# vnminin/phylomap

Hardware: AMD Instinct MI355X
Metric: stochastic-map realisations/sec (branches x sites sampled/s) (higher is better)
Workload: dtype f64; 1 GPU; C3: sumstatMCMC_bigtree sweep, 4-state Q, 10000-tip synthetic tree, Omega*mean(t_b)=4; n_states=4, n_tips=10000, branches=19998, replicas_total=16384, max_iters_provisioned=63, parallelism=replica-sharded x1 (weak), one RCCL all-reduce of the statistics

## Files before the change

### phylomap_amd/csrc/phm_device.h

```cpp
#pragma once

#include <hip/hip_runtime.h>
#include <stdint.h>

#define PHM_LOGTAB_QUAL __device__
#include "phm_logtab.h"

namespace phm {

constexpr uint32_t DERR_ZERO_PROB = 1u;
constexpr uint32_t DERR_CAPACITY  = 2u;
constexpr uint32_t DERR_UNIF_CAP  = 4u;
constexpr uint32_t DERR_SAMPLEONCE = 8u;

constexpr uint32_t ENT_NODE   = 0u;
constexpr uint32_t ENT_BSTATE = 1u << 30;
constexpr uint32_t ENT_BEXP   = 2u << 30;
constexpr uint32_t ENT_BUNIF  = 3u << 30;

#ifndef PHM_EXPERIMENT_PHILOX_ROUNDS
#define PHM_EXPERIMENT_PHILOX_ROUNDS 7
#endif
constexpr int PHILOX_ROUNDS = PHM_EXPERIMENT_PHILOX_ROUNDS;
__device__ __forceinline__ void philox4x32(uint32_t c0, uint32_t c1, uint32_t c2, uint32_t c3,
// ... 150 lines not shown
  for (int j = 1; j < NS - 1; ++j) { cum += p[j]; idx += (thr <= cum) ? 0 : 1; }
  return idx;
}

template <int NS>
__device__ __forceinline__ void matvec_u(const double* __restrict__ M, double (&v)[NS]) {
  double y[NS];
#pragma unroll
  for (int i = 0; i < NS; ++i) {
    double acc = M[i * NS] * v[0];
#pragma unroll
    for (int j = 1; j < NS; ++j) acc += M[i * NS + j] * v[j];
    y[i] = acc;
  }
#pragma unroll
  for (int i = 0; i < NS; ++i) v[i] = y[i];
}

template <int CTRL, int ROW_MASK>
__device__ __forceinline__ int dpp_max_step(int v) {
  const int o = __builtin_amdgcn_update_dpp(0, v, CTRL, ROW_MASK, 0xf, false);
  return o > v ? o : v;
}
__device__ __forceinline__ int wave_max_count(int v) {
  v = dpp_max_step<0x111, 0xf>(v);
  v = dpp_max_step<0x112, 0xf>(v);
  v = dpp_max_step<0x114, 0xf>(v);
  v = dpp_max_step<0x118, 0xf>(v);
  v = dpp_max_step<0x142, 0xa>(v);
  v = dpp_max_step<0x143, 0xc>(v);
  return __builtin_amdgcn_readlane(v, 63);
}

}
```

### phylomap_amd/csrc/phm_engine.cpp

```cpp
#include "phm_internal.h"

namespace {

int tree_levels(const phm::Schedule& s) {
  std::vector<int32_t> depth(s.n_node, 0);
  int levels = 1;
  for (const phm::DownStep& d : s.down)
    if (d.child >= 0) { depth[d.child] = depth[d.parent] + 1; levels = std::max(levels, depth[d.child] + 1); }
  return levels;
}
bool deep_tree(const phm::Schedule& s) {
  int lg2 = 0;
  while ((1 << lg2) < s.n_node + 1) ++lg2;
  return tree_levels(s) > 4 * lg2 + 32;
}

inline int narrow_auto_max_replicas(const phm::Schedule& s) {
  const int levels = tree_levels(s);
  const double E = (double)s.n_edge;
  const double cap = (0.0048 * levels + 6e-6 * E - 0.01) / (6.5e-7 * E);
  return (int)std::max(8.0, std::min(4096.0, cap));
}
constexpr int TILES_AUTO_MAX_REPLICAS = 262144;
inline int wbranch_auto_max_replicas(const phm::Schedule& s) {
// ... 514 lines not shown
    p.cnt = e->d_wb_cnt.as<double>(); p.rowbuf = e->d_nw_rowbuf.as<double>();
    p.dmap = e->d_nw_dmap.as<uint8_t>();
  }
  return PHM_OK;
}

inline int tiles_cnt_copies(int tiles) {
  int c = 1;
  while (c < 64 && c * tiles < 512) c *= 2;
  return c;
}

int32_t tiles_branch_group(int tiles, int n_edge) { return (int32_t)std::max<int64_t>(1, std::min<int64_t>(16, (int64_t)tiles * n_edge / 65536)); }

template <int NS>
void fill_tile_params(phm_engine* e, phm::TileParams<NS>& p, const phm_options& o) {
  fill_common(e, o, p);
  p.klong = e->nw_klong;
  p.tile0 = 0; p.tiles_part = e->tiles;
  p.group = tiles_branch_group(e->tiles, p.n_edge);
  p.n_groups = (p.n_edge + p.group - 1) / p.group;
  p.n_chunks = (p.n_groups + phm::TILES_CHUNK - 1) / phm::TILES_CHUNK;
  p.rows = e->nw_total_cap;
  p.up = e->d_up.as<phm::UpStep>();
  p.up_order = e->d_nw_up_order.as<int32_t>(); p.node_order = e->d_nw_node_order.as<int32_t>();
  p.branch_order = e->d_nw_border.as<int32_t>(); p.slot = e->d_tl_slot.as<int32_t>();
  p.cl_nodes = e->d_nw_cl_nodes.as<phm::ClusterNode>();
  p.cl_lvl_ptr = e->d_nw_cl_lvl_ptr.as<int32_t>(); p.cl_lvl_off = e->d_nw_cl_lvl_off.as<int32_t>();
  p.colL = e->d_nw_colL.as<double>(); p.rowL = e->d_nw_rowL.as<double>(); p.maskL = e->d_nw_maskL.as<double>();
  p.tips = e->d_tips.as<uint8_t>(); p.mcount = e->d_mcount.as<uint16_t>();
  p.dw[0] = e->d_dw0.as<double>(); p.dw[1] = e->d_dw1.as<double>();
  p.estate = e->d_tl_estate.as<uint8_t>(); p.PL = e->d_PL.as<double>(); p.nstate = e->d_nstate.as<uint8_t>();
  p.mstate = e->d_wt_mstate.p ? e->d_wt_mstate.as<uint8_t>() : nullptr;
  p.pdw = e->d_tl_pdw.as<double>(); p.pchunk = e->d_tl_pchunk.as<double>(); p.cnt = e->d_tl_cnt.as<uint32_t>();
  p.cnt_copies = tiles_cnt_copies(e->tiles);
  p.pseg = e->d_tl_pseg.as<uint32_t>(); p.segprev = e->d_tl_segprev.as<uint32_t>(); p.gseg = e->d_tl_gseg.p ? e->d_tl_gseg.as<uint32_t>() : nullptr;
}

int32_t tile_slots(phm_engine* e, const SlotPlan& sp) {
  const int E = e->sched.n_edge;
  e->tl_slot.assign(E + 1, 0);
  for (int b = 0; b < E; ++b) {
    if (sp.cap[b] >= (1 << 23)) return fail(PHM_ERR_UNSUPPORTED, "branch too long: a slot of the (tile, branch) mapping exceeds 4 GB");
    if (sp.off[b + 1] > 0x7fffff00ll / 64) return fail(PHM_ERR_UNSUPPORTED, "tree too large: dwell rows per replica tile exceed 32-bit indexing");
    e->tl_slot[b + 1] = (int32_t)sp.off[b + 1];
  }
  return PHM_OK;
}

int32_t tiles_setup(phm_engine* e, const phm_tree* x, const phm_model* model, const phm_options& o, int32_t max_iters) {
  const phm::Schedule& s = e->sched;
  const int E = s.n_edge, Nn = s.n_node, n = e->n, tiles = e->tiles;
  const SlotPlan sp = plan_slots(e, x, model->Omega, o, max_iters);
  if (int32_t st = tile_slots(e, sp)) return st;
  const int64_t rows = e->rows;
  single_tree_tips(e, x);

  const int n_chunks = (E + phm::TILES_CHUNK - 1) / phm::TILES_CHUNK;
  const size_t dw_bytes = sizeof(double) * (size_t)tiles * rows * 64;
  const size_t tab = (size_t)e->nw_klong * n * n;
  const size_t pdw_bytes = sizeof(double) * (size_t)tiles * E * n * 64;
  const size_t pl_bytes = sizeof(double) * (size_t)tiles * Nn * n * 64;
#ifndef PHM_TILES_LONG_SEGMENTS
#define PHM_TILES_LONG_SEGMENTS 48.0
#endif
  const bool long_paths = sp.max_seg > PHM_TILES_LONG_SEGMENTS;
  const size_t ms_bytes = long_paths ? (size_t)tiles * rows * 64 : 0;
  size_t free_b = 0, total_b = 0;
  HIPCHK(hipMemGetInfo(&free_b, &total_b));
  const int group = tiles_branch_group(tiles, E);
  const size_t gseg_bytes = group > 1 ? sizeof(uint32_t) * (size_t)tiles * ((E + group - 1) / group) * 64 : 0;
  const size_t need = 2 * dw_bytes + ms_bytes + pdw_bytes + gseg_bytes + pl_bytes + stats_bytes(e) + sizeof(double) * 3 * tab + (size_t)tiles * (4 * (size_t)E + Nn) * 64;
  if (int32_t st = check_hbm(need, free_b)) return st;
  HIPCHK(upload(e->d_up, s.up)); HIPCHK(upload(e->d_down, s.down));
  if (int32_t st = build_level_orders(e)) return st;
  HIPCHK(upload(e->d_nw_border, sp.order)); HIPCHK(upload(e->d_tl_slot, e->tl_slot));
  HIPCHK(e->d_nw_colL.alloc(sizeof(double) * tab)); HIPCHK(e->d_nw_rowL.alloc(sizeof(double) * tab));
  HIPCHK(e->d_nw_maskL.alloc(sizeof(double) * (size_t)e->nw_klong * 2 * n));
  HIPCHK(upload(e->d_tips, e->tips_host));
  HIPCHK(e->d_mcount.alloc(sizeof(uint16_t) * (size_t)tiles * E * 64));
  HIPCHK(e->d_dw0.alloc(dw_bytes)); HIPCHK(e->d_dw1.alloc(dw_bytes));
  if (long_paths) HIPCHK(e->d_wt_mstate.alloc(ms_bytes));
  HIPCHK(e->d_tl_estate.alloc((size_t)tiles * E * 64));
  HIPCHK(e->d_PL.alloc(pl_bytes));
  HIPCHK(e->d_nstate.alloc((size_t)tiles * Nn * 64));
  HIPCHK(e->d_tl_pdw.alloc(pdw_bytes));
  if (gseg_bytes) HIPCHK(e->d_tl_gseg.alloc(gseg_bytes));
  HIPCHK(e->d_tl_pchunk.alloc(sizeof(double) * (size_t)tiles * n_chunks * n * 64));
  HIPCHK(e->d_tl_cnt.alloc(sizeof(uint32_t) * (size_t)tiles * tiles_cnt_copies(tiles) * n * n * 64));
  HIPCHK(e->d_tl_pseg.alloc(sizeof(uint32_t) * (size_t)tiles * n_chunks * 64)); HIPCHK(e->d_tl_segprev.alloc(sizeof(uint32_t) * tiles));
  if (int32_t st = alloc_stats(e)) return st;
  e->bytes = (int64_t)(2 * dw_bytes + ms_bytes + pdw_bytes + gseg_bytes + pl_bytes + e->d_stats.bytes + e->d_red.bytes + e->d_mcount.bytes + e->d_tl_pchunk.bytes +
                       sizeof(double) * 3 * tab);
  HIPCHK(hipMemset(e->d_nstate.p, 0, e->d_nstate.bytes));
  HIPCHK(hipMemset(e->d_tl_cnt.p, 0, e->d_tl_cnt.bytes));
  if (int32_t st = init_tile_paths(e, x)) return st;
  {
    std::vector<uint32_t> segprev(tiles);
    for (int t = 0; t < tiles; ++t) segprev[t] = (uint32_t)((int64_t)x->map_off[E] * std::min(64, e->S - t * 64));
    HIPCHK(hipMemcpy(e->d_tl_segprev.p, segprev.data(), e->d_tl_segprev.bytes, hipMemcpyHostToDevice));
  }
  e->nw_tier_off.clear();
  const bool deep = deep_tree(s);
  if (e->dbg.level_groups >= 2 || (e->dbg.level_groups == 0 && (deep || (int64_t)tiles * Nn <= phm::TILES_CL_MAX_WORK))) {
    phm::ClusterPlan plan;
    if (e->dbg.level_groups == 3 || (e->dbg.level_groups == 0 && deep)) phm::build_cluster_plan(s, phm::TILES_CL_NODES, plan);
    else phm::build_band_plan(s, TILES_CL_BAND, plan);
    if (int32_t st = upload_cluster_plan(e, plan, false)) return st;
  }
  small_n(e, [&](auto& p) { fill_tile_params(e, p.tl, o); });
  return PHM_OK;
}

int32_t wtiles_setup(phm_engine* e, const phm_tree* x, const phm_model* model, const phm_options& o, int32_t max_iters) {
  const phm::Schedule& s = e->sched;
// ... 731 lines not shown
extern "C" {

int32_t phm_engine_dump(phm_engine* e, int32_t replica, int32_t* seg_count, double* seg_dwell, int32_t seg_cap,
                        int32_t* node_states, double* PL) {
  e = live(e);
  if (!e) return fail(PHM_ERR_STATE, "engine is NULL");
  if (e->dead) return dead_engine();
  if (replica < 0 || replica >= e->S) return fail(PHM_ERR_BAD_INPUT, "replica out of range");
  HIPCHK(hipSetDevice(e->device));
  HIPCHK(hipStreamSynchronize(e->last_stream));
  const bool branches = e->mapping == PHM_MAP_BRANCHES;
  const int padded = branches ? replica : e->pad_index(replica), L = branches ? 1 : 64, blk = padded / L, lane = padded % L;
  const phm::Schedule& s = e->scheds[e->n_trees > 1 ? blk / e->tpt : 0];
  const int E = s.n_edge, T = s.n_tips, n = e->n;
  if (branches) {
    std::vector<int32_t> mc(E);
    HIPCHK(hipMemcpy(mc.data(), e->d_nw_mcount.as<int32_t>() + (size_t)replica * E, sizeof(int32_t) * E, hipMemcpyDeviceToHost));
    if (seg_count) for (int b = 0; b < E; ++b) seg_count[b] = mc[b];
    if (seg_dwell) {
      std::vector<double> dw((size_t)e->nw_total_cap);
      const double* src = ((e->iters_done & 1) ? e->d_nw_dwB.as<double>() : e->d_nw_dwA.as<double>()) + (size_t)replica * e->nw_total_cap;
      HIPCHK(hipMemcpy(dw.data(), src, sizeof(double) * dw.size(), hipMemcpyDeviceToHost));
      for (int b = 0; b < E; ++b)
        for (int i = 0; i < std::min<int>(mc[b], seg_cap); ++i) seg_dwell[(size_t)b * seg_cap + i] = dw[(size_t)e->nw_off[b] + i];
    }
  } else {
    std::vector<uint16_t> mc((size_t)E * 64);
    HIPCHK(hipMemcpy(mc.data(), e->d_mcount.as<uint16_t>() + (size_t)blk * E * 64, sizeof(uint16_t) * mc.size(), hipMemcpyDeviceToHost));
    if (seg_count) for (int b = 0; b < E; ++b) seg_count[b] = mc[(size_t)b * 64 + lane];
    if (seg_dwell && e->mapping == PHM_MAP_TILES) {
      std::vector<double> dw((size_t)e->rows * 64);
      const double* src = ((e->iters_done & 1) ? e->d_dw1.as<double>() : e->d_dw0.as<double>()) + (size_t)blk * e->rows * 64;
      HIPCHK(hipMemcpy(dw.data(), src, sizeof(double) * dw.size(), hipMemcpyDeviceToHost));
      for (int b = 0; b < E; ++b)
        for (int i = 0; i < std::min<int>(mc[(size_t)b * 64 + lane], seg_cap); ++i)
          seg_dwell[(size_t)b * seg_cap + i] = dw[((size_t)e->tl_slot[b] + i) * 64 + lane];
    } else if (seg_dwell) {
      std::vector<double> dw((size_t)e->rows * 64);
      int32_t cur[2];
      HIPCHK(hipMemcpy(cur, e->d_cursor.as<int32_t>() + 2 * blk, sizeof cur, hipMemcpyDeviceToHost));
      const double* src = ((!e->ring && cur[0]) ? e->d_dw1.as<double>() : e->d_dw0.as<double>()) + (size_t)blk * e->rows * 64;
      HIPCHK(hipMemcpy(dw.data(), src, sizeof(double) * dw.size(), hipMemcpyDeviceToHost));
      size_t row = e->ring ? (size_t)cur[0] : 0;
      for (int k = 0; k < E; ++k) {
        const phm::DownStep& d = s.down[k];
        int m = std::min<int>(mc[(size_t)d.edge * 64 + lane], seg_cap);
        for (int i = 0; i < m; ++i) seg_dwell[(size_t)d.edge * seg_cap + i] = dw[((row + i) % (size_t)e->rows) * 64 + lane];
        int mx = 0;
        for (int l = 0; l < 64; ++l) mx = std::max<int>(mx, mc[(size_t)d.edge * 64 + l]);
        row += mx;
      }
    }
  }
  auto tip_state = [&](int t) -> int { return e->tips_per_replica ? e->tips_host[((size_t)blk * T + t) * L + lane] : e->tips_host[t]; };
  if (node_states) {
    std::vector<uint8_t> ns((size_t)s.n_node * L);
    HIPCHK(hipMemcpy(ns.data(), e->d_nstate.as<uint8_t>() + (size_t)blk * s.n_node * L, ns.size(), hipMemcpyDeviceToHost));
    for (int t = 0; t < T; ++t) node_states[t] = tip_state(t) + 1;
    for (int v = 0; v < s.n_node; ++v) node_states[T + v] = ns[(size_t)v * L + lane] + 1;
  }
  if (PL) {
    std::vector<double> pl((size_t)s.n_node * n * L);
    HIPCHK(hipMemcpy(pl.data(), e->d_PL.as<double>() + (size_t)blk * s.n_node * n * L, sizeof(double) * pl.size(), hipMemcpyDeviceToHost));
    for (int t = 0; t < T; ++t)
      for (int c = 0; c < n; ++c) PL[(size_t)t * n + c] = (c == tip_state(t)) ? 1.0 : 0.0;
    for (int v = 0; v < s.n_node; ++v)
      for (int c = 0; c < n; ++c)
        PL[(size_t)(T + v) * n + c] = (e->wide() && e->mapping == PHM_MAP_REPLICAS) ? pl[((size_t)v * L + lane) * n + c] : pl[((size_t)v * n + c) * L + lane];
  }
// ... 92 lines not shown
```

### phylomap_amd/csrc/phm_internal.h

```cpp
#pragma once

#include "../../include/phylomap_hip.h"

#include <hip/hip_runtime.h>

#include <algorithm>
#include <cmath>
#include <cstdio>
#include <chrono>
#include <cstdlib>
#include <cstring>
#include <memory>
#include <string>
#include <thread>
#include <vector>

#include "phm_exp.h"
#include "phm_mcmc.h"
#include "phm_mcmc_maps.h"
#include "phm_narrow.h"
#include "phm_qupdate.h"
#include "phm_sched.h"
#include "phm_tiles.h"
#include "phm_wbranch.h"
// ... 260 lines not shown
  bool recover = true;
  int recoveries = 0;
  bool dead = false;
  int n = 0, cols = 0, dcols = 0, variant = 0;
  std::vector<double> qparams;
  std::vector<std::vector<double>> qhist;
  double Omega = 0.0;
  std::vector<double> hB2, hBc, hscale, hpid;
  int S = 0, S_pad = 0, tiles = 0, max_iters = 0, iters_done = 0, ipl = 0;
  int reduce = 0, device = 0;
  bool normalise = false;
  phm::Schedule sched;
  std::vector<phm::Schedule> scheds;
  int n_trees = 1, S_tree = 0, tpt = 0;
  DevBuf d_roots;
  int rpt = 64;
  int pad_index(int r) const { return n_trees > 1 ? (r / S_tree) * tpt * 64 + r % S_tree : (r / rpt) * 64 + r % rpt; }
  std::vector<uint8_t> tips_host;
  bool tips_per_replica = false;
  int64_t rows = 0;
  DevBuf d_mask;
  DevBuf d_up, d_down, d_col, d_row, d_tips, d_mcount, d_dw0, d_dw1, d_cursor, d_PL, d_nstate, d_stats, d_err, d_seg, d_red, d_red_out;
  int32_t mapping = PHM_MAP_REPLICAS;
  bool wide() const { return n > 4; }
  template <int NS> struct SmallParams {
    phm::McmcParams<NS> rep;
    phm::NarrowParams<NS> br;
    phm::TileParams<NS> tl;
  };
  SmallParams<2> s2;
  SmallParams<3> s3;
  SmallParams<4> s4;
  bool ring = true;
  phm::WideParams pw;
  DevBuf d_B2, d_Bc, d_scale, d_pid;
  std::vector<int32_t> nw_walk_off;
  std::vector<int32_t> nw_tier_off;
  std::vector<int32_t> nw_up_off, nw_down_off;
  std::vector<int32_t> nw_node_off;
  std::vector<int64_t> nw_off;
  int nw_klong = 0;
  bool nw_cluster_async = false;
  int nw_n_wide = 0;
  int64_t nw_total_cap = 0;
  DevBuf d_nw_up_off, d_nw_down_off, d_nw_up_order, d_nw_down_order, d_nw_node_order, d_nw_border, d_nw_off, d_nw_colL, d_nw_rowL, d_nw_maskL, d_nw_mcount, d_nw_dwA, d_nw_dwB,
      d_nw_mstate, d_nw_mlen, d_nw_estate, d_nw_part, d_nw_rowbuf, d_nw_down_lv, d_nw_dmap, d_nw_dmap_edge, d_nw_walk_off, d_nw_edge_parent, d_nw_cl_nodes, d_nw_cl_item_off, d_nw_cl_lvl_ptr, d_nw_cl_lvl_off, d_ell_col, d_ell_val, d_ell2_col, d_ell2_val;
  DevBuf d_wb_cnt;
  phm::WideBranchParams pwb;
  std::vector<int32_t> tl_slot;
  DevBuf d_tl_slot, d_tl_pdw, d_tl_pchunk, d_tl_cnt, d_tl_estate, d_tl_pseg, d_tl_segprev, d_tl_gseg;
  static constexpr int MAX_PARTS = 4;
  hipStream_t part_stream[MAX_PARTS - 1] = {nullptr, nullptr, nullptr};
  hipEvent_t part_join[MAX_PARTS - 1] = {nullptr, nullptr, nullptr};
  int phase_parts = 1;
  void release_parts() {
    for (int i = 0; i < MAX_PARTS - 1; ++i) {
      if (part_stream[i]) { (void)hipStreamDestroy(part_stream[i]); part_stream[i] = nullptr; }
      if (part_join[i]) { (void)hipEventDestroy(part_join[i]); part_join[i] = nullptr; }
    }
  }
  phm::WtParams pwt;
  DevBuf d_wt_dwfx, d_wt_segacc, d_wt_B2, d_wt_totL, d_wt_pair_slot, d_wt_slot_col, d_wt_B2band, d_wt_mstate, d_wt_dwfx_tile, d_wt_cnt_tile;
  phm::WtBand wt_band;
  phm::WtSparseUp wt_sparse;
  DevBuf d_wt_coef;
  int sparse_req = 0;
// ... 91 lines not shown
```

### phylomap_amd/csrc/phm_mcmc_maps.hip

```cpp
#include "phm_mcmc_maps.h"

#include <algorithm>

namespace phm {

namespace {

constexpr int MM_BLOCK = 256;

template <class Draw, class Emit>
__device__ __forceinline__ void replay_branch(int m, int ps, int cs, const double* __restrict__ in, Stream& su, Draw draw, Emit emit) {
  int cur_s = (m == 1) ? cs : ps;
  double cur_len = in[0];
  for (int i = 1; i < m; ++i) {
    const int si = (i == m - 1) ? cs : draw(i, cur_s, su.draw_word((uint32_t)(i - 1)));
    const double di = in[(size_t)i * 64];
    if (si == cur_s) cur_len = cur_len + di;
    else { emit(cur_len, cur_s); cur_s = si; cur_len = di; }
  }
  emit(cur_len, cur_s);
}

template <int NS, int MODE>
__global__ __launch_bounds__(MM_BLOCK) void mcmc_maps_tiles_kernel(TileParams<NS> p, McmcMapsLaunch mp, int it) {
  __shared__ double s_B2[NS * NS];
  if (threadIdx.x < NS * NS) s_B2[threadIdx.x] = p.B2[threadIdx.x];
  __syncthreads();
  const int lane = threadIdx.x & 63;
  const int item = blockIdx.x * (MM_BLOCK / 64) + (threadIdx.x >> 6);
  if (item >= p.n_groups * p.n_tiles) return;
  const int tile = item % p.n_tiles, grp = item / p.n_tiles;
  const int r = tile * 64 + lane;
  if (r >= p.n_rep) return;
  const uint32_t rep = (uint32_t)(p.replica_offset + r);
  const int E = p.n_edge;
  const int q1 = min((grp + 1) * p.group, E);
  for (int q = grp * p.group; q < q1; ++q) {
    const int b = p.branch_order[q];
    const size_t eb = ((size_t)tile * E + b) * 64 + lane;
    const int m = p.mcount[eb];
    const int es = p.estate[eb];
    const int ps = es & 15, cs = es >> 4;
    const double* __restrict__ in = p.dw[it & 1] + ((size_t)tile * p.rows + p.slot[b]) * 64 + lane;
    Stream su;
    su.open(ENT_BSTATE | (uint32_t)b, (uint32_t)it, rep, p.seed_lo, p.seed_hi);
    const int64_t k = ((int64_t)r * mp.J + mp.j) * E + b;
    MapRow<MODE> mr;
    mr.begin(mp.dev, k);
    uint32_t err = 0;
    auto draw = [&](int i, int sprev, uint32_t word) -> int {
      const int kk = min(m - i - 1, p.klong - 1);
      const double* beta = p.colL + ((size_t)kk * NS + cs) * NS;
      double pr[NS];
#pragma unroll
      for (int c = 0; c < NS; ++c) pr[c] = s_B2[sprev * NS + c] * beta[c];
      return sample_cat<NS>(pr, u01(word), err);
    };
    replay_branch(m, ps, cs, in, su, draw, [&](double len, int s) { mr.emit(len, s); });
    mr.end(((size_t)mp.j * E + b) * p.n_rep_pad + r);
  }
}

template <int MODE>
__global__ __launch_bounds__(MM_BLOCK) void mcmc_maps_wtiles_kernel(WtParams p, McmcMapsLaunch mp, int it) {
  const int lane = threadIdx.x & 63;
  const int item = blockIdx.x * (MM_BLOCK / 64) + (threadIdx.x >> 6);
  if (item >= p.n_groups * p.n_tiles) return;
  const int tile = item % p.n_tiles, grp = item / p.n_tiles;
  const int r = tile * 64 + lane;
  if (r >= p.n_rep) return;
  const uint32_t rep = (uint32_t)(p.replica_offset + r);
  const int E = p.n_edge, n = p.n_states, ldt = p.ldt, nb = p.nblk;
  const int q1 = min((grp + 1) * p.group, E);
  for (int q = grp * p.group; q < q1; ++q) {
    const int b = p.branch_order[q];
    const size_t eb = ((size_t)tile * E + b) * 64 + lane;
    const int m = p.mcount[eb];
    const int es = p.estate[eb];
    const int ps = es & 255, cs = es >> 8;
    const double* __restrict__ in = p.dw[it & 1] + ((size_t)tile * p.rows + p.slot[b]) * 64 + lane;
    Stream su;
    su.open(ENT_BSTATE | (uint32_t)b, (uint32_t)it, rep, p.seed_lo, p.seed_hi);
    const int64_t k = ((int64_t)r * mp.J + mp.j) * E + b;
    MapRow<MODE> mr;
    mr.begin(mp.dev, k);
    auto draw = [&](int i, int sprev, uint32_t word) -> int {
      const int kk = min(m - i - 1, p.klong - 1);
      const double* __restrict__ blk = p.blkL + (((size_t)kk * n + sprev) * n + cs) * p.ldb;
      const double thr = u01(word) * blk[nb - 1];
      int b0 = 0;
      double cum = 0.0;
      for (int qq = 0; qq < nb - 1; ++qq) {
// ... 64 lines not shown
```

### phylomap_amd/csrc/phm_tiles.h

```cpp
#pragma once

#include <hip/hip_runtime.h>
#include <stdint.h>

#include <vector>

#include "phm_device.h"
#include "phm_sched.h"

namespace phm {

constexpr int TILES_BLOCK = 256;
constexpr int TILES_CHUNK = 64;
constexpr int TILES_PERSISTENT_WGS = 2048;
constexpr int TILES_KTAB = 24;
constexpr int TILES_CL_BLOCK = 512;
constexpr int TILES_CL_NODES = 256;
#ifndef TILES_CL_BAND
#define TILES_CL_BAND 8
#endif
constexpr int64_t TILES_CL_MAX_WORK = 65536;

template <int NS>
struct TileParams {
  int32_t n_tips, n_node, n_edge, root;
  int32_t n_tiles, n_rep, n_rep_pad, replica_offset;
  int32_t normalise, tips_per_replica, ks, tip_masks, reduce, n_cols;
  int32_t klong;
  int32_t group, n_groups;
  int32_t n_chunks;
  int32_t tile0, tiles_part;
  uint32_t seed_lo, seed_hi;
  int64_t rows;
  double B2[NS * NS], Bc[NS * NS], scale[NS], pid[NS];
  const UpStep* up;
  const int32_t* up_order;
  const int32_t* node_order;
  const ClusterNode* cl_nodes;
  const int32_t* cl_lvl_ptr;
  const int32_t* cl_lvl_off;
  const int32_t* branch_order;
  const int32_t* slot;
  const double* colL;
  const double* rowL;
  const double* maskL;
  const uint8_t* tips;
  uint16_t* mcount;
  double* dw[2];
  uint8_t* estate;
  uint8_t* mstate;
  double* PL;
  uint8_t* nstate;
  double* pdw;
  uint32_t* gseg;
  double* pchunk;
  uint32_t* cnt;
  int32_t cnt_copies;
  uint32_t* pseg;
  uint32_t* segprev;
  double* stats;
  uint32_t* err;
  unsigned long long* segcnt;
};

hipError_t launch_tiles_init(int n_edge, int n_tiles, int64_t rows, const int32_t* slot, const int32_t* map_off,
// ... 11 lines not shown
```

### phylomap_amd/csrc/phm_tiles.hip

```cpp
#include "phm_tiles.h"

#include <type_traits>

#include "phm_mcmc_maps.h"

namespace phm {

namespace {

template <int NS>
__device__ __forceinline__ void child_vec(const TileParams<NS>& p, const double* __restrict__ PLt,
                                          const uint8_t* __restrict__ tips_t, int child, int k, int lane, double (&v)[NS],
                                          uint32_t& err) {
  if (child < 0) {
    const int tip = ~child;
    const int st = p.tips_per_replica ? tips_t[tip * 64 + lane] : p.tips[tip];
    if (k >= p.klong) { err |= DERR_CAPACITY; k = p.klong - 1; }
    const double* src = (p.ks && p.tip_masks) ? p.maskL + ((size_t)k * 2 + (st & 1)) * NS : p.colL + ((size_t)k * NS + st) * NS;
#pragma unroll
    for (int c = 0; c < NS; ++c) v[c] = src[c];
  } else {
#pragma unroll
    for (int c = 0; c < NS; ++c) v[c] = PLt[(child * NS + c) * 64 + lane];
    for (int i = 0; i < k; ++i) matvec_u<NS>(p.Bc, v);
// ... 320 lines not shown
      node_finish<NS, decltype(k0)::value, decltype(k1)::value>(p, d, it, lane, err);
    });
  }
  if (err) atomicOr(p.err, err);
}

template <int NS>
__global__ __launch_bounds__(TILES_CL_BLOCK) void tiles_down_cluster_kernel(TileParams<NS> p, int it, int cl_begin, int n_cl, int with_root) {
  constexpr int W = TILES_CL_BLOCK / 64;
  const int lane = threadIdx.x & 63;
  const int wave = __builtin_amdgcn_readfirstlane(threadIdx.x >> 6);
  const int cl = cl_begin + (int)(blockIdx.x % (unsigned)n_cl);
  const int tile = (int)(blockIdx.x / (unsigned)n_cl);
  const int l0 = p.cl_lvl_ptr[cl], l1 = p.cl_lvl_ptr[cl + 1] - 1;
  uint32_t err = 0;
  if (with_root) {
    if (wave == 0) draw_root<NS>(p, tile, it, lane, err);
    __syncthreads();
  }
  for (int l = l1 - 1; l >= l0; --l) {
    const int i0 = p.cl_lvl_off[l], cnt = 2 * (p.cl_lvl_off[l + 1] - i0);
    for (int j = wave; j < cnt; j += W) {
      const ClusterNode nd = p.cl_nodes[i0 + (j >> 1)];
      down_edge<NS>(p, tile, it, nd.edge[j & 1], nd.parent, nd.child[j & 1], lane, err);
    }
    __syncthreads();
  }
  if (err) atomicOr(p.err, err);
}

template <int NS, bool KS, bool LONG>
__global__ __launch_bounds__(TILES_BLOCK, LONG ? 5 : (KS ? 7 : 8)) void tiles_branch_kernel(TileParams<NS> p, int it) {
  constexpr int NCNT = KS ? NS * NS : NS * (NS - 1);
  __shared__ double s_dw_all[(TILES_BLOCK / 64) * NS * 64];
  __shared__ uint16_t s_cnt_all[(TILES_BLOCK / 64) * NCNT * 64];
  __shared__ double s_B2[NS * NS], s_scale[NS];
  __shared__ double s_col[TILES_KTAB * NS * NS];
  __shared__ __align__(16) double s_ltab[2 * PHM_LOGTAB_N];
  const int lane = threadIdx.x & 63;
  const int wave = __builtin_amdgcn_readfirstlane(threadIdx.x >> 6);
  const int item = blockIdx.x * (TILES_BLOCK / 64) + wave;
  const uint32_t lane8 = (uint32_t)lane * 8u;
  const int ktab = min(TILES_KTAB, p.klong);
  for (int i = threadIdx.x; i < ktab * NS * NS; i += TILES_BLOCK) s_col[i] = p.colL[i];
  for (int i = threadIdx.x; i < 2 * PHM_LOGTAB_N; i += TILES_BLOCK) s_ltab[i] = logtab_entry(i);
  if (threadIdx.x < NS * NS) s_B2[threadIdx.x] = p.B2[threadIdx.x];
  if (threadIdx.x < NS) s_scale[threadIdx.x] = p.scale[threadIdx.x];
  __syncthreads();
  if (item >= p.n_groups * p.tiles_part) return;
  const int tile = p.tile0 + item % p.tiles_part;
  const int grp = item / p.tiles_part;
  double* s_dw = s_dw_all + wave * NS * 64;
  uint16_t* s_cnt = s_cnt_all + wave * NCNT * 64;
  const uint32_t rep = (uint32_t)(p.replica_offset + tile * 64 + lane);
  uint16_t* __restrict__ mct = p.mcount + (size_t)tile * p.n_edge * 64;
  uint32_t* gc = p.cnt + (((size_t)tile * p.cnt_copies + (grp & (p.cnt_copies - 1))) * NS * NS) * 64 + lane;
  uint32_t err = 0;
#pragma unroll
  for (int c = 0; c < NS; ++c) s_dw[c * 64 + lane] = 0.0;
#pragma unroll
  for (int c = 0; c < NCNT; ++c) s_cnt[c * 64 + lane] = (uint16_t)0;
  auto flush_counts = [&]() {
#pragma unroll
    for (int c = 0; c < NCNT; ++c) {
      const uint32_t v = s_cnt[c * 64 + lane];
      if (v) { atomicAdd(gc + c * 64, v); s_cnt[c * 64 + lane] = (uint16_t)0; }
    }
  };
  uint32_t pending = 0;
  uint32_t held = 0;
  const int q1 = min((grp + 1) * p.group, p.n_edge);
  for (int q = grp * p.group; q < q1; ++q) {
  const int b = p.branch_order[q];
  const int m = mct[b * 64 + lane];
  if (__any(pending + (uint32_t)m > 65535u)) { flush_counts(); pending = 0; }
  pending += (uint32_t)m;
  const int es = p.estate[((size_t)tile * p.n_edge + b) * 64 + lane];
  const int ps = es & 15, cs = es >> 4;
  const int roff = p.slot[b];
  const int cap = p.slot[b + 1] - roff;
  double* __restrict__ in = p.dw[it & 1] + ((size_t)tile * p.rows + roff) * 64;
  double* __restrict__ out = p.dw[(it & 1) ^ 1] + ((size_t)tile * p.rows + roff) * 64;
  auto IN = [&](int k) -> double& { return at(in, (uint32_t)k * 512u + lane8); };
  uint8_t* __restrict__ msrow = LONG ? p.mstate + ((size_t)tile * p.rows + roff) * 64 + lane : nullptr;
  auto MS = [&](int k) -> uint8_t& { return msrow[(uint32_t)k * 64u]; };

  Stream su, se;
  su.open(ENT_BSTATE | (uint32_t)b, (uint32_t)it, rep, p.seed_lo, p.seed_hi);
  se.open(ENT_BEXP | (uint32_t)b, (uint32_t)it, rep, p.seed_lo, p.seed_hi);
  const int mmax = wave_max_count(m);
  int mnew = 0;

  auto draw_state_w = [&](int i, int sprev, uint32_t word) -> int {
    int kk = m - i - 1;
    if (kk >= p.klong) { err |= DERR_CAPACITY; kk = p.klong - 1; }
    double pr[NS];
    {
      const double* beta = s_col + ((kk < ktab ? kk : ktab - 1) * NS + cs) * NS;
#pragma unroll
      for (int c = 0; c < NS; ++c) pr[c] = beta[c];
    }
    if (kk >= ktab) {
      const double* __restrict__ beta = p.colL + ((size_t)kk * NS + cs) * NS;
#pragma unroll
      for (int c = 0; c < NS; ++c) pr[c] = beta[c];
    }
#pragma unroll
    for (int c = 0; c < NS; ++c) pr[c] = s_B2[sprev * NS + c] * pr[c];
    return sample_cat<NS>(pr, u01(word), err);
  };
  auto draw_state = [&](int i, int sprev) -> int { return draw_state_w(i, sprev, su.draw_word((uint32_t)(i - 1))); };

  if (LONG || mmax <= 64) {
    uint64_t pk0 = 0, pk1 = 0;
    int w = 0;
    int cur_s = (m == 1) ? cs : ps;
    double first_len = 0.0, second_len = 0.0;
    double cur_len = IN(0);
    double dnext = (!LONG && m > 1) ? IN(1) : 0.0;
    double dq[4] = {0.0, 0.0, 0.0, 0.0}, bq[4][NS];
    auto beta_row = [&](int i, double (&bv)[NS]) {
      const int kk = min(max(m - i - 1, 0), p.klong - 1);
      const double* bl = s_col + ((kk < ktab ? kk : ktab - 1) * NS + cs) * NS;
#pragma unroll
      for (int c = 0; c < NS; ++c) bv[c] = bl[c];
      if (kk >= ktab) {
        const double* __restrict__ bg = p.colL + ((size_t)kk * NS + cs) * NS;
#pragma unroll
        for (int c = 0; c < NS; ++c) bv[c] = bg[c];
      }
    };
    if (LONG) {
#pragma unroll
      for (int q = 0; q < 4; ++q) {
#pragma unroll
        for (int c = 0; c < NS; ++c) bq[q][c] = 0.0;
        if (1 + q < m) { dq[q] = IN(1 + q); beta_row(1 + q, bq[q]); }
      }
    }
    for (int i0 = 1; i0 < mmax; i0 += 4) {
      uint32_t wd[4] = {0u, 0u, 0u, 0u};
      if (i0 < mmax - 1)
        philox4x32((uint32_t)((i0 - 1) >> 2), ENT_BSTATE | (uint32_t)b, (uint32_t)it, rep, p.seed_lo, p.seed_hi, wd);
#pragma unroll
      for (int q = 0; q < 4; ++q) {
      const int i = i0 + q;
      if (i < m) {
        int si;
        double di;
        if (LONG) {
          if (m - i - 1 >= p.klong) err |= DERR_CAPACITY;
          double pr[NS];
#pragma unroll
          for (int c = 0; c < NS; ++c) pr[c] = s_B2[cur_s * NS + c] * bq[q][c];
          si = (i == m - 1) ? cs : sample_cat<NS>(pr, u01(wd[q]), err);
          di = dq[q];
          if (i + 4 < m) { dq[q] = IN(i + 4); beta_row(i + 4, bq[q]); }
        } else {
          si = (i == m - 1) ? cs : draw_state_w(i, cur_s, wd[q]);
          di = dnext;
          if (i + 1 < m) dnext = IN(i + 1);
        }
        if (KS) s_cnt[(cur_s * NS + si) * 64 + lane] = (uint16_t)(s_cnt[(cur_s * NS + si) * 64 + lane] + 1u);
        if (si == cur_s) cur_len = cur_len + di;
        else {
          if (w == 0) first_len = cur_len; else if (w == 1) second_len = cur_len; else IN(w) = cur_len;
          if (LONG) MS(w) = (uint8_t)cur_s;
          else if (w < 32) pk0 |= (uint64_t)cur_s << (2 * w); else pk1 |= (uint64_t)cur_s << (2 * (w - 32));
          if (!KS) s_cnt[(cur_s * (NS - 1) + (si > cur_s ? si - 1 : si)) * 64 + lane] = (uint16_t)(s_cnt[(cur_s * (NS - 1) + (si > cur_s ? si - 1 : si)) * 64 + lane] + 1u);
          ++w; cur_s = si; cur_len = di;
        }
      }
      }
    }
    if (LONG) MS(w) = (uint8_t)cur_s;
    else if (w < 32) pk0 |= (uint64_t)cur_s << (2 * w); else pk1 |= (uint64_t)cur_s << (2 * (w - 32));
    const int first_s = (w == 0) ? cur_s : (LONG ? (int)MS(0) : (int)(pk0 & 3u));
    const int nmerged = w + 1;
    const double len0 = (w == 0) ? cur_len : first_len;

    int j = 0;
    int s = first_s;
    int snext = (LONG && nmerged > 1) ? (int)MS(1) : 0;
    double len = len0;
    double lnext = (nmerged > 1) ? ((w == 1) ? cur_len : second_len) : 0.0;
    double tot = 0.0, scale = s_scale[s], acc = s_dw[s * 64 + lane];
    bool stuck = false, done = false;
    for (uint32_t t0 = 0; __any(!done); t0 += 4) {
      uint32_t wd[4];
      philox4x32(t0 >> 2, ENT_BEXP | (uint32_t)b, (uint32_t)it, rep, p.seed_lo, p.seed_hi, wd);
#pragma unroll
      for (int q = 0; q < 4; ++q) {
        if (done) continue;
        double piece;
        bool adv;
        if (stuck || !(0.0 < len)) { stuck = true; piece = len; adv = true; }
        else {
          double rl = scale * neglog_u32(wd[q], s_ltab);
          if ((tot + rl) < len) { piece = rl; tot += rl; adv = false; }
          else { piece = len - tot; adv = true; }
        }
        if (mnew < cap) at(out, (uint32_t)mnew * 512u + lane8) = piece; else err |= DERR_CAPACITY;
        acc += piece;
        ++mnew;
        if (adv) {
          s_dw[s * 64 + lane] = acc;
          ++j;
          if (j >= nmerged) done = true;
          else {
            len = lnext;
            if (j + 1 < w) lnext = IN(j + 1); else lnext = cur_len;
            if (LONG) { s = snext; if (j + 1 < nmerged) snext = (int)MS(j + 1); }
            else s = (int)(((j < 32) ? (pk0 >> (2 * j)) : (pk1 >> (2 * (j - 32)))) & 3u);
            scale = s_scale[s]; tot = 0.0; acc = s_dw[s * 64 + lane];
          }
        }
      }
    }
  } else if (!LONG) {
    uint32_t edraw = 0;
    bool stuck = false;
    auto finalize = [&](int s, double len) {
      if (stuck || !(0.0 < len)) {
        stuck = true;
        if (mnew < cap) at(out, (uint32_t)mnew * 512u + lane8) = len; else err |= DERR_CAPACITY;
        s_dw[s * 64 + lane] += len;
        ++mnew;
        return;
      }
      const double scale = s_scale[s];
      double tot = 0.0;
      double acc = s_dw[s * 64 + lane];
      while (tot < len) {
        double rl = scale * neglog_u32(se.draw_word(edraw++), s_ltab);
        double piece;
        if ((tot + rl) < len) { piece = rl; tot += rl; }
        else { piece = len - tot; tot = len; }
        if (mnew < cap) at(out, (uint32_t)mnew * 512u + lane8) = piece; else err |= DERR_CAPACITY;
        acc += piece;
        ++mnew;
      }
      s_dw[s * 64 + lane] = acc;
    };
    int cur_s = (m == 1) ? cs : ps;
    double cur_len = IN(0);
    for (int i = 1; i <= m; ++i) {
      int si = -1;
      double di = 0.0;
      if (i < m) {
        si = (i == m - 1) ? cs : draw_state(i, cur_s);
        di = IN(i);
      }
      if (KS && si >= 0) s_cnt[(cur_s * NS + si) * 64 + lane] = (uint16_t)(s_cnt[(cur_s * NS + si) * 64 + lane] + 1u);
      if (si == cur_s) cur_len = cur_len + di;
      else {
        finalize(cur_s, cur_len);
        if (!KS && si >= 0) s_cnt[(cur_s * (NS - 1) + (si > cur_s ? si - 1 : si)) * 64 + lane] = (uint16_t)(s_cnt[(cur_s * (NS - 1) + (si > cur_s ? si - 1 : si)) * 64 + lane] + 1u);
        cur_s = si; cur_len = di;
      }
    }
  }
  if (mnew > cap) mnew = cap;
  if (mnew > 65535) { err |= DERR_CAPACITY; mnew = 65535; }
  mct[b * 64 + lane] = (uint16_t)mnew;
  held += (uint32_t)mnew;
  }
  flush_counts();
  if (p.group > 1) p.gseg[((size_t)tile * p.n_groups + grp) * 64 + lane] = held;

  double* pd = p.pdw + (((size_t)tile * p.n_edge + grp) * NS) * 64 + lane;
#pragma unroll
  for (int c = 0; c < NS; ++c) pd[c * 64] = s_dw[c * 64 + lane];
  if (err) atomicOr(p.err, err);
}

template <int NS>
__global__ __launch_bounds__(TILES_BLOCK) void tiles_chunk_kernel(TileParams<NS> p) {
  const int lane = threadIdx.x & 63;
  const int item = blockIdx.x * (TILES_BLOCK / 64) + __builtin_amdgcn_readfirstlane(threadIdx.x >> 6);
  if (item >= p.n_chunks * p.tiles_part) return;
  const int tile = p.tile0 + item / p.n_chunks, chunk = item % p.n_chunks;
  const int b0 = chunk * TILES_CHUNK, b1 = min(b0 + TILES_CHUNK, p.n_groups);
  double s[NS];
#pragma unroll
  for (int c = 0; c < NS; ++c) s[c] = 0.0;
  const double* src = p.pdw + ((size_t)tile * p.n_edge * NS) * 64 + lane;
  uint32_t segs = 0;
  if (p.group > 1) {
    const uint32_t* gs = p.gseg + ((size_t)tile * p.n_groups) * 64 + lane;
    for (int b = b0; b < b1; ++b) {
#pragma unroll
      for (int c = 0; c < NS; ++c) s[c] += src[((size_t)b * NS + c) * 64];
      segs += gs[(size_t)b * 64];
    }
  } else {
    for (int b = b0; b < b1; ++b)
#pragma unroll
// ... 93 lines not shown
}

__global__ void tiles_init_kernel(int n_edge, int n_tiles, int64_t rows, const int32_t* __restrict__ slot,
                                  const int32_t* __restrict__ map_off, const double* __restrict__ maps,
                                  double* __restrict__ dw0, uint16_t* __restrict__ mcount) {
  const int lane = threadIdx.x & 63;
  const int item = blockIdx.x * (blockDim.x / 64) + (threadIdx.x >> 6);
  if (item >= n_edge * n_tiles) return;
  const int tile = item / n_edge, b = item % n_edge;
  const int o = map_off[b], m = map_off[b + 1] - o;
  double* dst = dw0 + ((size_t)tile * rows + slot[b]) * 64 + lane;
  for (int i = 0; i < m; ++i) dst[(size_t)i * 64] = maps[o + i];
  mcount[((size_t)tile * n_edge + b) * 64 + lane] = (uint16_t)m;
}

}

hipError_t launch_tiles_init(int n_edge, int n_tiles, int64_t rows, const int32_t* slot, const int32_t* map_off,
                             const double* maps, double* dw0, uint16_t* mcount, hipStream_t stream) {
  const int64_t items = (int64_t)n_edge * n_tiles;
  hipLaunchKernelGGL(tiles_init_kernel, dim3((unsigned)((items + 3) / 4)), dim3(256), 0, stream, n_edge, n_tiles, rows, slot, map_off,
                     maps, dw0, mcount);
  return hipGetLastError();
}

template <int NS>
hipError_t launch_tiles_sweep(const TileParams<NS>& p, const std::vector<int32_t>& up_off,
                              const std::vector<int32_t>& node_off, const std::vector<int32_t>& tier_off, int it, hipStream_t stream,
                              hipEvent_t* phase_ev, const McmcMapsLaunch* maps) {
  constexpr int WPB = TILES_BLOCK / 64;
  auto blocks = [&](int64_t items) { return dim3((unsigned)((items + WPB - 1) / WPB)); };
  auto pblocks = [&](int64_t items) { return dim3((unsigned)std::min<int64_t>((items + WPB - 1) / WPB, TILES_PERSISTENT_WGS)); };
  auto mark = [&](int i) { if (phase_ev) (void)hipEventRecord(phase_ev[i], stream); };
  mark(0);
  if (p.cl_nodes) {
    const int n_tiers = (int)tier_off.size() - 1;
    for (int t = 0; t < n_tiers; ++t) {
      const int n_cl = tier_off[t + 1] - tier_off[t];
      if (p.mstate) hipLaunchKernelGGL((tiles_up_cluster_kernel<NS, true>), dim3((unsigned)((int64_t)n_cl * p.n_tiles)), dim3(TILES_CL_BLOCK), 0, stream, p, tier_off[t], n_cl);
      else hipLaunchKernelGGL((tiles_up_cluster_kernel<NS, false>), dim3((unsigned)((int64_t)n_cl * p.n_tiles)), dim3(TILES_CL_BLOCK), 0, stream, p, tier_off[t], n_cl);
    }
    mark(1);
    for (int t = n_tiers - 1; t >= 0; --t) {
      const int n_cl = tier_off[t + 1] - tier_off[t];
      hipLaunchKernelGGL(tiles_down_cluster_kernel<NS>, dim3((unsigned)((int64_t)n_cl * p.n_tiles)), dim3(TILES_CL_BLOCK), 0, stream, p, it, tier_off[t], n_cl,
                         t == n_tiers - 1 ? 1 : 0);
    }
  } else {
    for (size_t l = 0; l + 1 < up_off.size(); ++l) {
      const int n = up_off[l + 1] - up_off[l];
      if (n > 0) hipLaunchKernelGGL(tiles_up_kernel<NS>, blocks((int64_t)n * p.tiles_part), dim3(TILES_BLOCK), 0, stream, p, up_off[l], up_off[l + 1]);
    }
    mark(1);
    hipLaunchKernelGGL(tiles_root_kernel<NS>, blocks(p.tiles_part), dim3(TILES_BLOCK), 0, stream, p, it);
    for (size_t l = 0; l + 1 < node_off.size(); ++l) {
      const int n = node_off[l + 1] - node_off[l];
      if (n > 0) hipLaunchKernelGGL(tiles_down_kernel<NS>, pblocks((int64_t)n * p.tiles_part), dim3(TILES_BLOCK), 0, stream, p, it, node_off[l], node_off[l + 1]);
    }
  }
  mark(2);
  if (maps) {
    const hipError_t me = launch_mcmc_maps_tiles<NS>(p, *maps, it, stream);
    if (me != hipSuccess) return me;
  }
  if (p.mstate) {
    if (p.ks) hipLaunchKernelGGL((tiles_branch_kernel<NS, true, true>), blocks((int64_t)p.n_groups * p.tiles_part), dim3(TILES_BLOCK), 0, stream, p, it);
// ... 22 lines not shown
```

Baseline: 16.80 billion branch-site realisations/s.

## Compact per-branch dwell storage into dense wave-ranked rows for short paths

Short-path (non-LONG) mode now stores dwell segments compacted across the 64 replica lanes. Each row k holds only the lanes whose count exceeds k, and a lane's position comes from a ballot plus mbcnt prefix rank. This is meant to cut memory traffic and footprint when replicas have uneven segment counts, because the padded slots of lanes with fewer segments are no longer read or written. The cost is extra ballot/popcount work per step, wave-uniform loop bounds, an in-place rearrangement pass for paths longer than 64, and a host-side decoder for the new layout. Capacity checks also change to a wave-level limit.

Result: no change. 17.13 billion branch-site realisations/s, median of 6 (+1.9%).

```diff
diff --git a/phylomap_amd/csrc/phm_device.h b/phylomap_amd/csrc/phm_device.h
--- a/phylomap_amd/csrc/phm_device.h
+++ b/phylomap_amd/csrc/phm_device.h
@@ -206,4 +206,8 @@
   return __builtin_amdgcn_readlane(v, 63);
 }
 
-}
+__device__ __forceinline__ uint32_t lane_rank(uint64_t mask) {
+  return __builtin_amdgcn_mbcnt_hi((uint32_t)(mask >> 32), __builtin_amdgcn_mbcnt_lo((uint32_t)mask, 0u));
+}
+
+}
diff --git a/phylomap_amd/csrc/phm_engine.cpp b/phylomap_amd/csrc/phm_engine.cpp
--- a/phylomap_amd/csrc/phm_engine.cpp
+++ b/phylomap_amd/csrc/phm_engine.cpp
@@ -570,6 +570,7 @@
   p.dw[0] = e->d_dw0.as<double>(); p.dw[1] = e->d_dw1.as<double>();
   p.estate = e->d_tl_estate.as<uint8_t>(); p.PL = e->d_PL.as<double>(); p.nstate = e->d_nstate.as<uint8_t>();
   p.mstate = e->d_wt_mstate.p ? e->d_wt_mstate.as<uint8_t>() : nullptr;
+  p.dense = e->tl_dense ? 1 : 0;
   p.pdw = e->d_tl_pdw.as<double>(); p.pchunk = e->d_tl_pchunk.as<double>(); p.cnt = e->d_tl_cnt.as<uint32_t>();
   p.cnt_copies = tiles_cnt_copies(e->tiles);
   p.pseg = e->d_tl_pseg.as<uint32_t>(); p.segprev = e->d_tl_segprev.as<uint32_t>(); p.gseg = e->d_tl_gseg.p ? e->d_tl_gseg.as<uint32_t>() : nullptr;
@@ -619,6 +620,10 @@
   HIPCHK(e->d_mcount.alloc(sizeof(uint16_t) * (size_t)tiles * E * 64));
   HIPCHK(e->d_dw0.alloc(dw_bytes)); HIPCHK(e->d_dw1.alloc(dw_bytes));
   if (long_paths) HIPCHK(e->d_wt_mstate.alloc(ms_bytes));
+  e->tl_dense = !long_paths;
+  if (e->tl_dense) {
+    HIPCHK(hipMemset(e->d_dw0.p, 0, dw_bytes)); HIPCHK(hipMemset(e->d_dw1.p, 0, dw_bytes));
+  }
   HIPCHK(e->d_tl_estate.alloc((size_t)tiles * E * 64));
   HIPCHK(e->d_PL.alloc(pl_bytes));
   HIPCHK(e->d_nstate.alloc((size_t)tiles * Nn * 64));
@@ -1416,9 +1421,16 @@
       std::vector<double> dw((size_t)e->rows * 64);
       const double* src = ((e->iters_done & 1) ? e->d_dw1.as<double>() : e->d_dw0.as<double>()) + (size_t)blk * e->rows * 64;
       HIPCHK(hipMemcpy(dw.data(), src, sizeof(double) * dw.size(), hipMemcpyDeviceToHost));
-      for (int b = 0; b < E; ++b)
-        for (int i = 0; i < std::min<int>(mc[(size_t)b * 64 + lane], seg_cap); ++i)
-          seg_dwell[(size_t)b * seg_cap + i] = dw[((size_t)e->tl_slot[b] + i) * 64 + lane];
+      for (int b = 0; b < E; ++b) {
+        size_t before = 0;
+        for (int i = 0; i < std::min<int>(mc[(size_t)b * 64 + lane], seg_cap); ++i) {
+          if (!e->tl_dense) { seg_dwell[(size_t)b * seg_cap + i] = dw[((size_t)e->tl_slot[b] + i) * 64 + lane]; continue; }
+          size_t rank = 0, cells = 0;
+          for (int l = 0; l < 64; ++l) { const bool in_row = mc[(size_t)b * 64 + l] > i; cells += in_row; rank += in_row && l < lane; }
+          seg_dwell[(size_t)b * seg_cap + i] = dw[(size_t)e->tl_slot[b] * 64 + before + rank];
+          before += cells;
+        }
+      }
     } else if (seg_dwell) {
       std::vector<double> dw((size_t)e->rows * 64);
       int32_t cur[2];
diff --git a/phylomap_amd/csrc/phm_internal.h b/phylomap_amd/csrc/phm_internal.h
--- a/phylomap_amd/csrc/phm_internal.h
+++ b/phylomap_amd/csrc/phm_internal.h
@@ -316,6 +316,7 @@
   SmallParams<3> s3;
   SmallParams<4> s4;
   bool ring = true;
+  bool tl_dense = false;
   phm::WideParams pw;
   DevBuf d_B2, d_Bc, d_scale, d_pid;
   std::vector<int32_t> nw_walk_off;
diff --git a/phylomap_amd/csrc/phm_mcmc_maps.hip b/phylomap_amd/csrc/phm_mcmc_maps.hip
--- a/phylomap_amd/csrc/phm_mcmc_maps.hip
+++ b/phylomap_amd/csrc/phm_mcmc_maps.hip
@@ -21,6 +21,26 @@
   emit(cur_len, cur_s);
 }
 
+template <class Draw, class Emit>
+__device__ __forceinline__ void replay_branch_dense(int m, bool live, int ps, int cs, const double* __restrict__ slot, Stream& su, Draw draw, Emit emit) {
+  const int mmax = wave_max_count(m);
+  uint64_t mrow = __builtin_amdgcn_ballot_w64(0 < m);
+  uint32_t before = 0;
+  int cur_s = (m == 1) ? cs : ps;
+  double cur_len = (0 < m) ? slot[before + lane_rank(mrow)] : 0.0;
+  for (int i = 1; i < mmax; ++i) {
+    before += (uint32_t)__builtin_popcountll(mrow);
+    mrow = __builtin_amdgcn_ballot_w64(i < m);
+    if (live && i < m) {
+      const int si = (i == m - 1) ? cs : draw(i, cur_s, su.draw_word((uint32_t)(i - 1)));
+      const double di = slot[before + lane_rank(mrow)];
+      if (si == cur_s) cur_len = cur_len + di;
+      else { emit(cur_len, cur_s); cur_s = si; cur_len = di; }
+    }
+  }
+  if (live) emit(cur_len, cur_s);
+}
+
 template <int NS, int MODE>
 __global__ __launch_bounds__(MM_BLOCK) void mcmc_maps_tiles_kernel(TileParams<NS> p, McmcMapsLaunch mp, int it) {
   __shared__ double s_B2[NS * NS];
@@ -31,7 +51,8 @@
   if (item >= p.n_groups * p.n_tiles) return;
   const int tile = item % p.n_tiles, grp = item / p.n_tiles;
   const int r = tile * 64 + lane;
-  if (r >= p.n_rep) return;
+  const bool live = r < p.n_rep;
+  if (!p.dense && !live) return;
   const uint32_t rep = (uint32_t)(p.replica_offset + r);
   const int E = p.n_edge;
   const int q1 = min((grp + 1) * p.group, E);
@@ -41,12 +62,12 @@
     const int m = p.mcount[eb];
     const int es = p.estate[eb];
     const int ps = es & 15, cs = es >> 4;
-    const double* __restrict__ in = p.dw[it & 1] + ((size_t)tile * p.rows + p.slot[b]) * 64 + lane;
+    const double* __restrict__ slot = p.dw[it & 1] + ((size_t)tile * p.rows + p.slot[b]) * 64;
     Stream su;
     su.open(ENT_BSTATE | (uint32_t)b, (uint32_t)it, rep, p.seed_lo, p.seed_hi);
     const int64_t k = ((int64_t)r * mp.J + mp.j) * E + b;
     MapRow<MODE> mr;
-    mr.begin(mp.dev, k);
+    mr.begin(mp.dev, k, live);
     uint32_t err = 0;
     auto draw = [&](int i, int sprev, uint32_t word) -> int {
       const int kk = min(m - i - 1, p.klong - 1);
@@ -56,8 +77,9 @@
       for (int c = 0; c < NS; ++c) pr[c] = s_B2[sprev * NS + c] * beta[c];
       return sample_cat<NS>(pr, u01(word), err);
     };
-    replay_branch(m, ps, cs, in, su, draw, [&](double len, int s) { mr.emit(len, s); });
-    mr.end(((size_t)mp.j * E + b) * p.n_rep_pad + r);
+    if (p.dense) replay_branch_dense(m, live, ps, cs, slot, su, draw, [&](double len, int s) { mr.emit(len, s); });
+    else replay_branch(m, ps, cs, slot + lane, su, draw, [&](double len, int s) { mr.emit(len, s); });
+    if (live) mr.end(((size_t)mp.j * E + b) * p.n_rep_pad + r);
   }
 }
 
diff --git a/phylomap_amd/csrc/phm_tiles.h b/phylomap_amd/csrc/phm_tiles.h
--- a/phylomap_amd/csrc/phm_tiles.h
+++ b/phylomap_amd/csrc/phm_tiles.h
@@ -31,6 +31,7 @@
   int32_t n_chunks;
   int32_t tile0, tiles_part;
   uint32_t seed_lo, seed_hi;
+  int32_t dense;
   int64_t rows;
   double B2[NS * NS], Bc[NS * NS], scale[NS], pid[NS];
   const UpStep* up;
diff --git a/phylomap_amd/csrc/phm_tiles.hip b/phylomap_amd/csrc/phm_tiles.hip
--- a/phylomap_amd/csrc/phm_tiles.hip
+++ b/phylomap_amd/csrc/phm_tiles.hip
@@ -376,6 +376,7 @@
 template <int NS, bool KS, bool LONG>
 __global__ __launch_bounds__(TILES_BLOCK, LONG ? 5 : (KS ? 7 : 8)) void tiles_branch_kernel(TileParams<NS> p, int it) {
   constexpr int NCNT = KS ? NS * NS : NS * (NS - 1);
+  constexpr bool DENSE = !LONG;
   __shared__ double s_dw_all[(TILES_BLOCK / 64) * NS * 64];
   __shared__ uint16_t s_cnt_all[(TILES_BLOCK / 64) * NCNT * 64];
   __shared__ double s_B2[NS * NS], s_scale[NS];
@@ -415,10 +416,11 @@
   uint32_t held = 0;
   const int q1 = min((grp + 1) * p.group, p.n_edge);
   for (int q = grp * p.group; q < q1; ++q) {
-  const int b = p.branch_order[q];
+  const int b = __builtin_amdgcn_readfirstlane(p.branch_order[q]);
   const int m = mct[b * 64 + lane];
-  if (__any(pending + (uint32_t)m > 65535u)) { flush_counts(); pending = 0; }
-  pending += (uint32_t)m;
+  const int mmax = wave_max_count(m);
+  if (pending + (uint32_t)mmax > 65535u) { flush_counts(); pending = 0; }
+  pending += (uint32_t)mmax;
   const int es = p.estate[((size_t)tile * p.n_edge + b) * 64 + lane];
   const int ps = es & 15, cs = es >> 4;
   const int roff = p.slot[b];
@@ -426,13 +428,14 @@
   double* __restrict__ in = p.dw[it & 1] + ((size_t)tile * p.rows + roff) * 64;
   double* __restrict__ out = p.dw[(it & 1) ^ 1] + ((size_t)tile * p.rows + roff) * 64;
   auto IN = [&](int k) -> double& { return at(in, (uint32_t)k * 512u + lane8); };
+  auto cell = [&](uint64_t mask, uint32_t before) -> uint32_t { return (before + lane_rank(mask)) * 8u; };
+  auto PARK = [&](int k) -> double& { return DENSE ? at(out, ((uint32_t)(cap + 1 - k) * 64u + (uint32_t)lane) * 8u) : IN(k); };
   uint8_t* __restrict__ msrow = LONG ? p.mstate + ((size_t)tile * p.rows + roff) * 64 + lane : nullptr;
   auto MS = [&](int k) -> uint8_t& { return msrow[(uint32_t)k * 64u]; };
 
   Stream su, se;
   su.open(ENT_BSTATE | (uint32_t)b, (uint32_t)it, rep, p.seed_lo, p.seed_hi);
   se.open(ENT_BEXP | (uint32_t)b, (uint32_t)it, rep, p.seed_lo, p.seed_hi);
-  const int mmax = wave_max_count(m);
   int mnew = 0;
 
   auto draw_state_w = [&](int i, int sprev, uint32_t word) -> int {
@@ -455,13 +458,29 @@
   };
   auto draw_state = [&](int i, int sprev) -> int { return draw_state_w(i, sprev, su.draw_word((uint32_t)(i - 1))); };
 
+  if (DENSE && mmax > 64) {
+    uint32_t before = 0;
+    for (int k = 0; k < mmax; ++k) before += (uint32_t)__builtin_popcountll(__builtin_amdgcn_ballot_w64(k < m));
+    for (int k = mmax - 1; k >= 0; --k) {
+      const uint64_t mk = __builtin_amdgcn_ballot_w64(k < m);
+      before -= (uint32_t)__builtin_popcountll(mk);
+      if (k < m) { const double v = at(in, cell(mk, before)); IN(k) = v; }
+    }
+  }
   if (LONG || mmax <= 64) {
     uint64_t pk0 = 0, pk1 = 0;
     int w = 0;
     int cur_s = (m == 1) ? cs : ps;
     double first_len = 0.0, second_len = 0.0;
-    double cur_len = IN(0);
-    double dnext = (!LONG && m > 1) ? IN(1) : 0.0;
+    uint64_t mrow = DENSE ? __builtin_amdgcn_ballot_w64(0 < m) : 0ull;
+    uint32_t ibefore = 0;
+    double cur_len = DENSE ? ((0 < m) ? at(in, cell(mrow, ibefore)) : 0.0) : IN(0);
+    double dnext = 0.0;
+    if (DENSE) {
+      ibefore += (uint32_t)__builtin_popcountll(mrow);
+      mrow = __builtin_amdgcn_ballot_w64(1 < m);
+      if (1 < m) dnext = at(in, cell(mrow, ibefore));
+    }
     double dq[4] = {0.0, 0.0, 0.0, 0.0}, bq[4][NS];
     auto beta_row = [&](int i, double (&bv)[NS]) {
       const int kk = min(max(m - i - 1, 0), p.klong - 1);
@@ -489,6 +508,10 @@
 #pragma unroll
       for (int q = 0; q < 4; ++q) {
       const int i = i0 + q;
+      if (DENSE) {
+        ibefore += (uint32_t)__builtin_popcountll(mrow);
+        mrow = __builtin_amdgcn_ballot_w64(i + 1 < m);
+      }
       if (i < m) {
         int si;
         double di;
@@ -503,12 +526,12 @@
         } else {
           si = (i == m - 1) ? cs : draw_state_w(i, cur_s, wd[q]);
           di = dnext;
-          if (i + 1 < m) dnext = IN(i + 1);
+          if (i + 1 < m) dnext = at(in, cell(mrow, ibefore));
         }
         if (KS) s_cnt[(cur_s * NS + si) * 64 + lane] = (uint16_t)(s_cnt[(cur_s * NS + si) * 64 + lane] + 1u);
         if (si == cur_s) cur_len = cur_len + di;
         else {
-          if (w == 0) first_len = cur_len; else if (w == 1) second_len = cur_len; else IN(w) = cur_len;
+          if (w == 0) first_len = cur_len; else if (w == 1) second_len = cur_len; else PARK(w) = cur_len;
           if (LONG) MS(w) = (uint8_t)cur_s;
           else if (w < 32) pk0 |= (uint64_t)cur_s << (2 * w); else pk1 |= (uint64_t)cur_s << (2 * (w - 32));
           if (!KS) s_cnt[(cur_s * (NS - 1) + (si > cur_s ? si - 1 : si)) * 64 + lane] = (uint16_t)(s_cnt[(cur_s * (NS - 1) + (si > cur_s ? si - 1 : si)) * 64 + lane] + 1u);
@@ -529,13 +552,18 @@
     double len = len0;
     double lnext = (nmerged > 1) ? ((w == 1) ? cur_len : second_len) : 0.0;
     double tot = 0.0, scale = s_scale[s], acc = s_dw[s * 64 + lane];
-    bool stuck = false, done = false;
-    for (uint32_t t0 = 0; __any(!done); t0 += 4) {
+    bool stuck = false;
+    uint32_t obefore = 0;
+    const uint32_t olimit = DENSE ? 64u * (uint32_t)(cap - max(0, wave_max_count(w) - 2)) : 0u;
+    for (uint32_t t0 = 0; __any(j < nmerged); t0 += 4) {
       uint32_t wd[4];
       philox4x32(t0 >> 2, ENT_BEXP | (uint32_t)b, (uint32_t)it, rep, p.seed_lo, p.seed_hi, wd);
 #pragma unroll
       for (int q = 0; q < 4; ++q) {
-        if (done) continue;
+        const uint64_t mout = DENSE ? __builtin_amdgcn_ballot_w64(j < nmerged) : 0ull;
+        const uint32_t nout = (uint32_t)__builtin_popcountll(mout);
+        const bool room = DENSE ? (t0 + (uint32_t)q < (uint32_t)cap && obefore + nout <= olimit) : false;
+        if (j < nmerged) {
         double piece;
         bool adv;
         if (stuck || !(0.0 < len)) { stuck = true; piece = len; adv = true; }
@@ -544,21 +572,23 @@
           if ((tot + rl) < len) { piece = rl; tot += rl; adv = false; }
           else { piece = len - tot; adv = true; }
         }
-        if (mnew < cap) at(out, (uint32_t)mnew * 512u + lane8) = piece; else err |= DERR_CAPACITY;
+        if (DENSE) { if (room) at(out, cell(mout, obefore)) = piece; else err |= DERR_CAPACITY; }
+        else if (mnew < cap) at(out, (uint32_t)mnew * 512u + lane8) = piece; else err |= DERR_CAPACITY;
         acc += piece;
         ++mnew;
         if (adv) {
           s_dw[s * 64 + lane] = acc;
           ++j;
-          if (j >= nmerged) done = true;
-          else {
+          if (j < nmerged) {
             len = lnext;
-            if (j + 1 < w) lnext = IN(j + 1); else lnext = cur_len;
+            if (j + 1 < w) lnext = PARK(j + 1); else lnext = cur_len;
             if (LONG) { s = snext; if (j + 1 < nmerged) snext = (int)MS(j + 1); }
             else s = (int)(((j < 32) ? (pk0 >> (2 * j)) : (pk1 >> (2 * (j - 32)))) & 3u);
             scale = s_scale[s]; tot = 0.0; acc = s_dw[s * 64 + lane];
           }
         }
+        }
+        obefore += nout;
       }
     }
   } else if (!LONG) {
@@ -603,10 +633,20 @@
         cur_s = si; cur_len = di;
       }
     }
+    if (DENSE) {
+      const int mc = min(mnew, cap);
+      const int mcmax = wave_max_count(mc);
+      uint32_t before = 0;
+      for (int k = 0; k < mcmax; ++k) {
+        const uint64_t mk = __builtin_amdgcn_ballot_w64(k < mc);
+        if (k < mc) { const double v = at(out, (uint32_t)k * 512u + lane8); at(out, cell(mk, before)) = v; }
+        before += (uint32_t)__builtin_popcountll(mk);
+      }
+    }
   }
   if (mnew > cap) mnew = cap;
   if (mnew > 65535) { err |= DERR_CAPACITY; mnew = 65535; }
-  mct[b * 64 + lane] = (uint16_t)mnew;
+  at(mct, (uint32_t)b * 128u + (uint32_t)lane * 2u) = (uint16_t)mnew;
   held += (uint32_t)mnew;
   }
   flush_counts();
@@ -766,6 +806,7 @@
   auto blocks = [&](int64_t items) { return dim3((unsigned)((items + WPB - 1) / WPB)); };
   auto pblocks = [&](int64_t items) { return dim3((unsigned)std::min<int64_t>((items + WPB - 1) / WPB, TILES_PERSISTENT_WGS)); };
   auto mark = [&](int i) { if (phase_ev) (void)hipEventRecord(phase_ev[i], stream); };
+  if ((p.dense != 0) != (p.mstate == nullptr)) return hipErrorInvalidValue;
   mark(0);
   if (p.cl_nodes) {
     const int n_tiers = (int)tier_off.size() - 1;
```
